# WGLab/NanoMod

Hardware: AMD Instinct MI355X
Metric: genomic positions/sec (KS + Stouffer) (higher is better)
Workload: dtype f32 keys / f64 p-values; 1 GPU; BASELINE.json configs[1]: E. coli 4.6 Mb: 4600000 positions in total (4600000 per GPU), 200 v 200 reads/position, KS + weighted Stouffer window=5; preset=ecoli, positions_total=4600000, positions_per_gpu=4600000, n0=200, n1=200, layout=fixed stride, ties=few, spread_milli=0, outlier_permille=0, rccl_ranks=0, ks_d=float form, bit for bit, parallelism=one GPU, no collective

## Files before the change

nanomod_amd/csrc/ks_rank.hpp:

```cpp
#pragma once
#include <hip/hip_runtime.h>
#include <stdint.h>
#include <type_traits>
#include "rank_stats_packed.hpp"
#include "packed_sort_i16.hpp"
#include "item_claim.hpp"

namespace nmod {

static __device__ const float kKsBig4[4] = {3.4028234663852886e38f, 3.4028234663852886e38f, 3.4028234663852886e38f, 3.4028234663852886e38f};
static __device__ const unsigned kKsInf4[4] = {0x7f800000u, 0x7f800000u, 0x7f800000u, 0x7f800000u};
static __device__ const unsigned kKsPad16[4] = {0x7fff7fffu, 0x7fff7fffu, 0x7fff7fffu, 0x7fff7fffu};

__host__ __device__ constexpr bool ks_packed_sort(int R, int LG, int DTYPE) { return DTYPE == 1 && R == 16 && (LG == 8 || LG == 16); }

template <int R, int LG>
struct KsLayout {
  static constexpr int C = R * LG;
  static constexpr int ROW = LG + 1;
  static constexpr int REGION = R * ROW;
  static constexpr int LAST = (R - 1) * ROW + LG - 1;
  static constexpr int END = LG;
  __device__ static __forceinline__ int word(int i) { return __mul24(i & (R - 1), ROW) + i / R; }
};

__host__ __device__ constexpr int ks_rank_pos_words(int R, int LG) {
  int w = 2 * R * (LG + 1);
  if (LG <= 16) while ((w & 31) != LG) ++w;
  return w;
}

template <typename T>
__device__ __forceinline__ T ks_global_load(const void* p) {
  typedef const T __attribute__((address_space(1)))* GlobalPtr;
  return *(GlobalPtr)(p);
}

typedef float KsF4v __attribute__((ext_vector_type(4)));
typedef short KsS4v __attribute__((ext_vector_type(4)));
typedef KsF4v KsF4 __attribute__((aligned(4)));
typedef KsS4v KsS4 __attribute__((aligned(2)));

template <int R, int LG, int DTYPE>
struct KsRows {
  using T = typename std::conditional<DTYPE == 0, float, int16_t>::type;
  using V4 = typename std::conditional<DTYPE == 0, KsF4, KsS4>::type;
  static constexpr int NK = R / 4;
  V4 v[NK];
  T s[3];

  __device__ __forceinline__ void request(const void* sig, int64_t off, int n, int gl) {
    const T* row = reinterpret_cast<const T*>(sig) + off;
    const T* dummy = ks_packed_sort(R, LG, DTYPE) ? reinterpret_cast<const T*>(kKsPad16) : reinterpret_cast<const T*>(kKsInf4);
    const bool long_row = n >= 4;
#pragma unroll
    for (int k = 0; k < NK; ++k) {
      const int idx = k * (4 * LG) + 4 * gl;
      const int t = n - idx;
      const T* p = (long_row && t > 0) ? row + ((t >= 4) ? idx : n - 4) : dummy;
      v[k] = ks_global_load<V4>(p);
    }
    s[0] = s[1] = s[2] = T(0);
    if (__ballot(!long_row && n > 0) != 0ull) {
#pragma unroll
      for (int e = 0; e < 3; ++e)
        if (!long_row && gl == 0 && e < n) s[e] = ks_global_load<T>(row + e);
    }
  }

  __device__ __forceinline__ void finish(float (&x)[R], int n, int gl) const {
    const float inf = __builtin_inff();
    const bool long_row = n >= 4;
#pragma unroll
    for (int k = 0; k < NK; ++k) {
      const int idx = k * (4 * LG) + 4 * gl;
      const int t = long_row ? n - idx : 0;
      if constexpr (DTYPE == 0) {
        x[4 * k + 0] = v[k].x; x[4 * k + 1] = v[k].y; x[4 * k + 2] = v[k].z; x[4 * k + 3] = v[k].w;
        if (__ballot(t > 0 && t < 4) != 0ull) {
          x[4 * k + 0] = (t >= 4 || t <= 0) ? x[4 * k + 0] : inf;
          x[4 * k + 1] = (t >= 3 || t <= 0) ? x[4 * k + 1] : inf;
          x[4 * k + 2] = (t >= 2 || t <= 0) ? x[4 * k + 2] : inf;
        }
      } else {
        x[4 * k + 0] = (t >= 4) ? (float)v[k].x : inf;
        x[4 * k + 1] = (t >= 3) ? (float)v[k].y : inf;
        x[4 * k + 2] = (t >= 2) ? (float)v[k].z : inf;
        x[4 * k + 3] = (t >= 1) ? (float)v[k].w : inf;
      }
    }
    if (__ballot(!long_row && n > 0) != 0ull) {
#pragma unroll
      for (int e = 0; e < 3; ++e) x[e] = (!long_row && gl == 0 && e < n) ? (float)s[e] : x[e];
    }
  }

  __device__ __forceinline__ void finish_packed(unsigned (&p)[8], int n, int gl) const {
    static_assert(R == 16, "packed rows: 16 keys per lane");
    const bool long_row = n >= 4;
#pragma unroll
    for (int k = 0; k < NK; ++k) {
      p[2 * k] = ((unsigned)(unsigned short)v[k].y << 16) | (unsigned)(unsigned short)v[k].x;
      p[2 * k + 1] = ((unsigned)(unsigned short)v[k].w << 16) | (unsigned)(unsigned short)v[k].z;
      const int idx = k * (4 * LG) + 4 * gl;
      const int t = long_row ? n - idx : 0;
      if (__ballot(t > 0 && t < 4) != 0ull) {
        if (t == 3) p[2 * k] = (p[2 * k] & 0xffff0000u) | 0x7fffu;
        if (t == 2 || t == 1) p[2 * k] = 0x7fff7fffu;
        if (t == 1) p[2 * k + 1] = (p[2 * k + 1] & 0xffff0000u) | 0x7fffu;
      }
    }
    if (__ballot(!long_row && n > 0) != 0ull) {
      if (!long_row && gl == 0) {
        const unsigned s0 = (0 < n) ? (unsigned)(unsigned short)s[0] : 0x7fffu;
        const unsigned s1 = (1 < n) ? (unsigned)(unsigned short)s[1] : 0x7fffu;
        const unsigned s2 = (2 < n) ? (unsigned)(unsigned short)s[2] : 0x7fffu;
        p[0] = (s1 << 16) | s0;
        p[1] = (0x7fffu << 16) | s2;
      }
    }
  }
};

template <int LG>
__device__ __forceinline__ unsigned seg_allmax_u32(unsigned v) {
  v = max(v, (unsigned)dpp_i<NMOD_QP(1, 0, 3, 2), 0xf, 0xf, true>(0, (int)v));
  v = max(v, (unsigned)dpp_i<NMOD_QP(2, 3, 0, 1), 0xf, 0xf, true>(0, (int)v));
  v = max(v, (unsigned)dpp_i<kDppRowHalfMirror, 0xf, 0xf, true>(0, (int)v));
  if constexpr (LG >= 16) v = max(v, (unsigned)dpp_i<kDppRowMirror, 0xf, 0xf, true>(0, (int)v));
  if constexpr (LG >= 32) v = max(v, (unsigned)__builtin_amdgcn_ds_swizzle((int)v, 0x401F));
  if constexpr (LG == 64) v = max(__builtin_amdgcn_readlane(v, 0), __builtin_amdgcn_readlane(v, 32));
  return v;
}

template <int LG>
__device__ __forceinline__ unsigned seg_exscan_add_u32(unsigned v, int gl) {
  unsigned inc = v;
  auto step = [&](auto tag, int dist) {
    constexpr int C = decltype(tag)::value;
    unsigned t = (unsigned)dpp_i<C, 0xf, 0xf, true>(0, (int)inc);
    inc += (gl >= dist) ? t : 0u;
  };
  step(std::integral_constant<int, kDppRowShr + 1>{}, 1);
  step(std::integral_constant<int, kDppRowShr + 2>{}, 2);
  step(std::integral_constant<int, kDppRowShr + 4>{}, 4);
  if constexpr (LG >= 16) step(std::integral_constant<int, kDppRowShr + 8>{}, 8);
  if constexpr (LG >= 32) {
    unsigned t = (unsigned)dpp_i<kDppRowBcast15, 0xA>(0, (int)inc);
    inc += ((gl & 16) != 0) ? t : 0u;
  }
  if constexpr (LG == 64) {
    unsigned t = (unsigned)dpp_i<kDppRowBcast31, 0xC>(0, (int)inc);
    inc += (gl >= 32) ? t : 0u;
  }
  return inc - v;
}

template <int R, int LG>
__device__ __forceinline__ void seg_sort_any(float (&x)[R], const LaneSel& sel, int lane) {
  seg_sort<R, (LG == 64 ? 32 : LG)>(x, sel, lane);
  if constexpr (LG == 64) merge_lanes<R, 64>(x, sel, lane);
}

template <int R, int LG, bool LE, bool FULL = true>
__device__ __forceinline__ const float* ks_search(const float* base, float x) {
  using Lay = KsLayout<R, LG>;
  const float* p = base;
  bool all = false;
  if constexpr (FULL) {
    const float last = base[Lay::LAST];
    all = LE ? (last <= x) : (last < x);
  }
#pragma unroll
  for (int hc = LG / 2; hc >= 1; hc >>= 1) {
    const float t = p[(R - 1) * Lay::ROW + hc - 1];
    const bool right = LE ? (t <= x) : (t < x);
    p = right ? p + hc : p;
  }
#pragma unroll
  for (int h = R / 2; h >= 1; h >>= 1) {
    const float t = p[(h - 1) * Lay::ROW];
    const bool right = LE ? (t <= x) : (t < x);
    p = right ? p + h * Lay::ROW : p;
  }
  return all ? base + Lay::END : p;
}

struct KsTops { float hi, lo0, lo1, last; };
template <int R, int LG>
__device__ __forceinline__ KsTops ks_tops(const float* base) {
  using Lay = KsLayout<R, LG>;
  auto uni = [](float v) { return __int_as_float(__builtin_amdgcn_readfirstlane(__float_as_int(v))); };
  KsTops t;
  t.hi = uni(base[(R - 1) * Lay::ROW + LG / 2 - 1]);
  t.lo0 = uni(base[(R - 1) * Lay::ROW + LG / 4 - 1]);
  t.lo1 = uni(base[(R - 1) * Lay::ROW + LG / 2 + LG / 4 - 1]);
  t.last = uni(base[Lay::LAST]);
  return t;
}
template <int R, int LG>
__device__ __forceinline__ const float* ks_search_tops(const float* base, float x, const KsTops& t) {
  using Lay = KsLayout<R, LG>;
  static_assert(LG >= 4, "two row levels");
  const bool all = t.last < x;
  const bool r1 = t.hi < x;
  const float t2 = r1 ? t.lo1 : t.lo0;
  const bool r2 = t2 < x;
  const float* p = base + (r1 ? LG / 2 : 0) + (r2 ? LG / 4 : 0);
#pragma unroll
  for (int hc = LG / 8; hc >= 1; hc >>= 1) {
    const float v = p[(R - 1) * Lay::ROW + hc - 1];
    p = (v < x) ? p + hc : p;
  }
#pragma unroll
  for (int h = R / 2; h >= 1; h >>= 1) {
    const float v = p[(h - 1) * Lay::ROW];
    p = (v < x) ? p + h * Lay::ROW : p;
  }
  return all ? base + Lay::END : p;
}

__device__ __forceinline__ double fmax_numbers(double a, double b) {
  double r;
  asm("v_max_f64 %0, %1, %2" : "=v"(r) : "v"(a), "v"(b));
  return r;
}

template <int LG>
__device__ __forceinline__ double seg_allmax_f64(double v) {
  v = fmax_numbers(v, dpp_f64_row(v, 0)); v = fmax_numbers(v, dpp_f64_row(v, 1)); v = fmax_numbers(v, dpp_f64_row(v, 2));
  if constexpr (LG >= 16) v = fmax_numbers(v, dpp_f64_row(v, 3));
  if constexpr (LG >= 32) v = fmax(v, xor16_f64(v));
  if constexpr (LG == 64) v = wave_max_f64(v);
  return v;
}

__device__ __forceinline__ double hist_exact_quot(int c, double n, double r) {
  const double dc = (double)c;
  const double q0 = __dmul_rn(dc, r);
  const double rem = __fma_rn(-q0, n, dc);
  return __fma_rn(rem, r, q0);
}

template <int LG>
__device__ __forceinline__ void seg_moments_packed16(const unsigned (&p)[8], int n, int gl, double& mean, double& m2, double rcp_n = 0.0) {
  int s1 = 0;
  double s2 = 0.0;
#pragma unroll
  for (int j = 0; j < 8; ++j) {
    const int lo = (int)(short)(p[j] & 0xffffu), hi = (int)p[j] >> 16;
    s1 += lo + hi;
    const double dl = (double)lo, dh = (double)hi;
    s2 = __fma_rn(dl, dl, s2);
    s2 = __fma_rn(dh, dh, s2);
  }
  int valid = 0;
#pragma unroll
  for (int k = 0; k < 4; ++k) valid += min(max(n - (k * 4 * LG + 4 * gl), 0), 4);
  valid = (n >= 4) ? valid : ((gl == 0) ? n : 0);
  const int npad = 16 - valid;
  s1 -= 32767 * npad;
  s2 -= 1073676289.0 * (double)npad;
  unsigned v = (unsigned)s1;
  v += (unsigned)dpp_i<NMOD_QP(1, 0, 3, 2), 0xf, 0xf, true>(0, (int)v);
  v += (unsigned)dpp_i<NMOD_QP(2, 3, 0, 1), 0xf, 0xf, true>(0, (int)v);
  v += (unsigned)dpp_i<kDppRowHalfMirror, 0xf, 0xf, true>(0, (int)v);
  if constexpr (LG >= 16) v += (unsigned)dpp_i<kDppRowMirror, 0xf, 0xf, true>(0, (int)v);
  const double S1 = (double)(int)v;
  const double S2 = seg_allsum_f64<LG>(s2);
  const double dn = (double)n;
  const double num = __fma_rn(dn, S2, -S1 * S1);
  const double rn = (rcp_n != 0.0) ? rcp_n : 1.0 / dn;
  mean = S1 * rn * 1e-3;
  m2 = num * rn * 1e-6;
}

template <int R, int LG, int DTYPE, bool FLAGS = false>
__global__ __launch_bounds__(64 * kWavesPerBlock, (R <= 16 ? 4 : 2))
void ks_rank_kernel(RankStatsArgs args) {
  static_assert(LG == 8 || LG == 16 || LG == 32 || LG == 64, "lanes per sorted group");
  static_assert(R >= 8 && R <= 32 && (R & (R - 1)) == 0, "registers per lane");
  constexpr int PW = 64 / LG;
  using Lay = KsLayout<R, LG>;
  constexpr int ROW = Lay::ROW;
  constexpr int POS_WORDS = ks_rank_pos_words(R, LG);
  constexpr int HIST_OFF = Lay::REGION;
  extern __shared__ __attribute__((aligned(16))) float lds_all[];

  const int lane = threadIdx.x & 63;
  const int wave = __builtin_amdgcn_readfirstlane(threadIdx.x >> 6);
  const int gl = lane & (LG - 1);
  const int slot = lane / LG;
  float* keys = lds_all + (wave * PW + slot) * POS_WORDS;
  unsigned* hist = reinterpret_cast<unsigned*>(keys + HIST_OFF);
  const int e0 = gl * R;

  const float inf = __builtin_inff();
  LaneSel sel;
#pragma unroll
  for (int b = 0; b < 6; ++b) sel.s[b] = ((lane >> b) & 1) ? inf : -inf;
  for (int r = gl; r < R; r += LG) keys[r * ROW + Lay::END] = inf;
  const bool uniform = args.stride0 > 0 && args.stride1 > 0;
  double* recip = reinterpret_cast<double*>(lds_all + kWavesPerBlock * PW * POS_WORDS);
  if (uniform && threadIdx.x == 0) {
    const int64_t a0 = args.stride0 < args.stride1 ? args.stride0 : args.stride1;
    const int64_t a1 = args.stride0 < args.stride1 ? args.stride1 : args.stride0;
    recip[0] = 1.0 / (double)a0; recip[1] = 1.0 / (double)a1;
  }
  __syncthreads();

  int64_t count = args.npos;
  const int32_t* list = nullptr;
  if (args.alt_gates != nullptr && args.alt_gates[args.class_id] != 0) {
    count = args.alt_meta[args.class_id];
    list = args.alt_list + args.alt_meta[kClassStride + args.class_id];
  } else if (args.pos_list) {
    count = args.class_meta[args.class_id];
    list = args.pos_list + args.class_meta[kClassStride + args.class_id];
  }
  const int64_t items = (count + PW - 1) / PW;
  const int64_t wave_global = (int64_t)blockIdx.x * kWavesPerBlock + wave;
  const int64_t wave_stride = (int64_t)gridDim.x * kWavesPerBlock;

  struct Item { bool valid, swap; int m, q; int64_t pos, off_s, off_q; };
  const uint32_t items32 = (uint32_t)items;
  auto describe = [&](uint32_t it) {
    Item d;
    const uint32_t li = min(it, items32) * PW + slot;
    d.valid = li < (uint32_t)count;
    d.pos = d.valid ? (list ? (int64_t)list[li] : (int64_t)li) : 0;
    int64_t o0 = 0, o1 = 0; int n0 = 0, n1 = 0;
    if (d.valid) {
      if (args.stride0 > 0) { o0 = (int64_t)((uint64_t)(uint32_t)d.pos * (uint64_t)(uint32_t)args.stride0); n0 = (int)args.stride0; }
      else { o0 = args.off0[d.pos]; n0 = (int)(args.off0[d.pos + 1] - o0); }
      if (args.stride1 > 0) { o1 = (int64_t)((uint64_t)(uint32_t)d.pos * (uint64_t)(uint32_t)args.stride1); n1 = (int)args.stride1; }
      else { o1 = args.off1[d.pos]; n1 = (int)(args.off1[d.pos + 1] - o1); }
    }
    d.swap = n1 < n0;
    d.m = d.swap ? n1 : n0; d.q = d.swap ? n0 : n1;
    d.off_s = d.swap ? o1 : o0; d.off_q = d.swap ? o0 : o1;
    return d;
  };
  const float big = 3.4028234663852886e38f;
  using Q4Raw = typename std::conditional<DTYPE == 0, KsF4, KsS4>::type;
  using Q1Raw = typename std::conditional<DTYPE == 0, float, int16_t>::type;
  auto load_q4 = [&](const void* sig, int64_t off, int idx, bool have) -> Q4Raw {
    using T = Q1Raw;
    const T* src = have ? reinterpret_cast<const T*>(sig) + off + idx : reinterpret_cast<const T*>(kKsBig4);
    return ks_global_load<Q4Raw>(src);
  };
  auto q4_values = [&](float (&xq)[4], const Q4Raw& t, bool have) {
    if constexpr (DTYPE == 0) {
      (void)have;
      xq[0] = t.x; xq[1] = t.y; xq[2] = t.z; xq[3] = t.w;
    } else {
      xq[0] = have ? (float)t.x : big; xq[1] = have ? (float)t.y : big;
      xq[2] = have ? (float)t.z : big; xq[3] = have ? (float)t.w : big;
    }
  };
  auto load_q1 = [&](const void* sig, int64_t off, int idx, bool have) -> Q1Raw {
    using T = Q1Raw;
    return ks_global_load<T>(have ? reinterpret_cast<const T*>(sig) + off + idx : reinterpret_cast<const T*>(kKsBig4));
  };
  auto q1_value = [&](Q1Raw v, bool have) -> float {
    if constexpr (DTYPE == 0) { (void)have; return v; }
    else return have ? (float)v : big;
  };

  ItemWalk walk;
  const uint32_t it_first = walk.begin(item_claim_plan<uint32_t>((uint32_t)items, (uint32_t)wave_stride, args.strided_items != 0),
                                      (uint32_t)wave_global, (uint32_t)wave_stride, args.claim + args.class_id, lane);
  Item cur = describe(it_first);
  constexpr bool PACKED = ks_packed_sort(R, LG, DTYPE);
  float x[R];
  unsigned pk[8];
  {
    KsRows<R, LG, DTYPE> first;
    first.request(cur.swap ? args.sig1 : args.sig0, cur.off_s, cur.m, gl);
    if constexpr (PACKED) first.finish_packed(pk, cur.m, gl);
    else first.finish(x, cur.m, gl);
  }
  __builtin_amdgcn_s_waitcnt(0x0F70);
  walk.collect();

  for (uint32_t it = it_first, it_next; it < items32; it = it_next) {
    const bool valid = cur.valid;
    const int64_t pos = cur.pos;
    const int m = cur.m, q = cur.q;
    const void* sig_q = cur.swap ? args.sig0 : args.sig1;
    const int64_t off_q = cur.off_q;

    const int full = q / (4 * LG);
    const int tail = (q - full * (4 * LG) + LG - 1) / LG;
    int full_w = full, tail_w = tail;
    if constexpr (PW > 1) {
      full_w = 0; tail_w = 0;
#pragma unroll
      for (int s = 0; s < PW; ++s) {
        full_w = max(full_w, __builtin_amdgcn_readlane(full, s * LG));
        tail_w = max(tail_w, __builtin_amdgcn_readlane(tail, s * LG));
      }
    } else {
      full_w = __builtin_amdgcn_readfirstlane(full);
      tail_w = __builtin_amdgcn_readfirstlane(tail);
    }
    int slots = (full_w * 4 + tail_w) * LG;
    bool coop = false;
    if constexpr (PW > 1) {
      int coop_cost = 0;
#pragma unroll
      for (int sl = 0; sl < PW; ++sl) {
        const int qs = __builtin_amdgcn_readlane(q, sl * LG);
        const int fs = qs / 256;
        coop_cost += fs * 4 + (qs - fs * 256 + 63) / 64;
      }
      coop = coop_cost < full_w * 4 + tail_w;
    }
    it_next = walk.next(it, lane);
    const Item nxt = describe(it_next);
    KsRows<R, LG, DTYPE> rows_next;
    rows_next.request(nxt.swap ? args.sig1 : args.sig0, nxt.off_s, nxt.m, gl);
    constexpr bool PIPE_COOP = LG == 8;
    auto row_of_slot = [&](int sl, const void*& sg, int64_t& of, int& qn) {
      const int src = sl * LG;
      auto rl64 = [&](unsigned long long v) {
        const unsigned lo = (unsigned)__builtin_amdgcn_readlane((int)(unsigned)v, src);
        const unsigned hi = (unsigned)__builtin_amdgcn_readlane((int)(unsigned)(v >> 32), src);
        return ((unsigned long long)hi << 32) | (unsigned long long)lo;
      };
      sg = reinterpret_cast<const void*>((uintptr_t)rl64((unsigned long long)(uintptr_t)sig_q));
      of = (int64_t)rl64((unsigned long long)off_q);
      qn = __builtin_amdgcn_readlane(q, src);
    };
    const void* sig_c = sig_q; int64_t off_c = off_q; int q_c = q;
    int idx_a = 4 * gl, idx_t = full * (4 * LG) + gl;
    bool have_a = !coop && 0 < full, have_t = !coop && idx_t < q;
    if constexpr (PIPE_COOP) {
      if (coop) {
        row_of_slot(0, sig_c, off_c, q_c);
        idx_a = 4 * lane; idx_t = (q_c / 256) * 256 + lane; have_a = q_c >= 256; have_t = idx_t < q_c;
      }
    }
    Q4Raw ra = load_q4(sig_c, off_c, idx_a, have_a);
    Q1Raw rt = load_q1(sig_c, off_c, idx_t, have_t);

    if constexpr (PACKED) {
      seg_sort_packed16<LG>(pk, lane);
      unpack_sorted16<LG>(pk, x);
    } else {
      seg_sort_any<R, LG>(x, sel, lane);
    }
#pragma unroll
    for (int r = 0; r < R; ++r) keys[r * ROW + gl] = x[r];
    if constexpr (PACKED) {
      const int real = m - e0;
#pragma unroll
      for (int r = 0; r < R; ++r)
        if (r >= real) keys[r * ROW + gl] = inf;
    }
#pragma unroll
    for (int r = 0; r < R; ++r) hist[r * ROW + gl] = 0u;
    if (gl == LG - 1) hist[Lay::END] = 0u;
    __builtin_amdgcn_fence(__ATOMIC_RELEASE, "wavefront");
    __builtin_amdgcn_wave_barrier();

    const bool s_full = __ballot(m == Lay::C) != 0ull;

    auto rank_and_count = [&](auto nv_tag, auto full_tag, const float* kbase, const float* xq) {
      constexpr int NV = decltype(nv_tag)::value;
      constexpr bool FULL = decltype(full_tag)::value;
      const float* lp[NV];
#pragma unroll
      for (int e = 0; e < NV; ++e) lp[e] = ks_search<R, LG, false, FULL>(kbase, xq[e]);
      unsigned inc[NV];
#pragma unroll
      for (int e = 0; e < NV; ++e) inc[e] = (*lp[e] == xq[e]) ? 0x10001u : 0x10000u;
#pragma unroll
      for (int e = 0; e < NV; ++e) atomicAdd(reinterpret_cast<unsigned*>(const_cast<float*>(lp[e])) + HIST_OFF, inc[e]);
    };

    [[maybe_unused]] auto rank_and_count_tops = [&](auto nv_tag, const float* kbase, const KsTops& tops, const float* xq) {
      constexpr int NV = decltype(nv_tag)::value;
      const float* lp[NV];
#pragma unroll
      for (int e = 0; e < NV; ++e) lp[e] = ks_search_tops<R, LG>(kbase, xq[e], tops);
      unsigned inc[NV];
#pragma unroll
      for (int e = 0; e < NV; ++e) inc[e] = (*lp[e] == xq[e]) ? 0x10001u : 0x10000u;
#pragma unroll
      for (int e = 0; e < NV; ++e) atomicAdd(reinterpret_cast<unsigned*>(const_cast<float*>(lp[e])) + HIST_OFF, inc[e]);
    };

    __builtin_amdgcn_s_waitcnt(0x0F70);
    walk.collect();
    if (!coop) {
#pragma unroll 1
      for (int c = 0; c < full_w; ++c) {
        const Q4Raw rb = load_q4(sig_q, off_q, (c + 1) * (4 * LG) + 4 * gl, c + 1 < full);
        float xa[4];
        q4_values(xa, ra, c < full);
        if (s_full) rank_and_count(std::integral_constant<int, 4>{}, std::true_type{}, keys, xa);
        else rank_and_count(std::integral_constant<int, 4>{}, std::false_type{}, keys, xa);
        ra = rb;
      }
#pragma unroll 1
      for (int c = 0; c < tail_w; ++c) {
        float xq[1] = {q1_value(rt, full * (4 * LG) + c * LG + gl < q)};
        const int idx = full * (4 * LG) + (c + 1) * LG + gl;
        rt = load_q1(sig_q, off_q, idx, idx < q);
        if (s_full) rank_and_count(std::integral_constant<int, 1>{}, std::true_type{}, keys, xq);
        else rank_and_count(std::integral_constant<int, 1>{}, std::false_type{}, keys, xq);
      }
    } else {
      const int cfull = q / 256;
      slots = (cfull * 4 + (q - cfull * 256 + 63) / 64) * 64;
      if constexpr (PIPE_COOP) {
#pragma unroll 1
      for (int sl = 0; sl < PW; ++sl) {
        const void* sig_n = sig_c; int64_t off_n = off_c; int q_n = 0;
        if (sl + 1 < PW) row_of_slot(sl + 1, sig_n, off_n, q_n);
        const int nfs = q_n / 256;
        const Q4Raw na = load_q4(sig_n, off_n, 4 * lane, nfs > 0);
        const Q1Raw nt = load_q1(sig_n, off_n, nfs * 256 + lane, nfs * 256 + lane < q_n);
        const float* kb = lds_all + (wave * PW + sl) * POS_WORDS;
        const int fs = q_c / 256, ts = (q_c - fs * 256 + 63) / 64;
        const KsTops tops = ks_tops<R, LG>(kb);
#pragma unroll 2
        for (int c = 0; c < fs; ++c) {
          const Q4Raw rb = load_q4(sig_c, off_c, min(c + 1, fs - 1) * 256 + 4 * lane, true);
          float xq[4];
          q4_values(xq, ra, true);
          rank_and_count_tops(std::integral_constant<int, 4>{}, kb, tops, xq);
          ra = rb;
        }
#pragma unroll 1
        for (int c = 0; c < ts; ++c) {
          const int idx_now = fs * 256 + c * 64 + lane;
          const Q1Raw r1 = load_q1(sig_c, off_c, idx_now + 64, idx_now + 64 < q_c);
          float xq[1] = {q1_value(rt, idx_now < q_c)};
          rank_and_count_tops(std::integral_constant<int, 1>{}, kb, tops, xq);
          rt = r1;
        }
        sig_c = sig_n; off_c = off_n; q_c = q_n; ra = na; rt = nt;
      }
      } else {
#pragma unroll 1
      for (int sl = 0; sl < PW; ++sl) {
        const int src = sl * LG;
        const int qs = __builtin_amdgcn_readlane(q, src);
        const unsigned long long sp = (unsigned long long)(uintptr_t)sig_q;
        auto rl64 = [&](unsigned long long v) {
          const unsigned lo = (unsigned)__builtin_amdgcn_readlane((int)(unsigned)v, src);
          const unsigned hi = (unsigned)__builtin_amdgcn_readlane((int)(unsigned)(v >> 32), src);
          return ((unsigned long long)hi << 32) | (unsigned long long)lo;
        };
        const void* sigs = reinterpret_cast<const void*>((uintptr_t)rl64(sp));
        const int64_t offs = (int64_t)rl64((unsigned long long)off_q);
        const float* kb = lds_all + (wave * PW + sl) * POS_WORDS;
        const int fs = qs / 256, ts = (qs - fs * 256 + 63) / 64;
#pragma unroll 1
        for (int c = 0; c < fs; ++c) {
          const int idx = c * 256 + 4 * lane;
          float xq[4];
          q4_values(xq, load_q4(sigs, offs, idx, true), true);
          rank_and_count(std::integral_constant<int, 4>{}, std::true_type{}, kb, xq);
        }
#pragma unroll 1
        for (int c = 0; c < ts; ++c) {
          const int idx = fs * 256 + c * 64 + lane;
          float xq[1] = {q1_value(load_q1(sigs, offs, idx, idx < qs), idx < qs)};
          rank_and_count(std::integral_constant<int, 1>{}, std::true_type{}, kb, xq);
        }
      }
      }
    }
    __builtin_amdgcn_fence(__ATOMIC_RELEASE, "wavefront");
    __builtin_amdgcn_wave_barrier();
    if (gl == 0) { const unsigned extra = (unsigned)(slots - q); hist[Lay::word(m)] -= extra << 16; }
    __builtin_amdgcn_fence(__ATOMIC_RELEASE, "wavefront");
    __builtin_amdgcn_wave_barrier();

    unsigned h[R];
#pragma unroll
    for (int r = 0; r < R - 1; ++r) h[r] = hist[(r + 1) * ROW + gl];
    h[R - 1] = hist[gl + 1];
    const unsigned h0 = hist[0];
    unsigned tot = 0;
#pragma unroll
    for (int r = 0; r < R; ++r) tot += h[r];
    const unsigned cum = seg_exscan_add_u32<LG>(tot, gl) + h0;
    unsigned best = 0;
    float s_own[R];
#pragma unroll
    for (int r = 0; r < R; ++r) s_own[r] = keys[r * ROW + gl];
    const float s_next = keys[gl + 1];
    const bool tie_lane = ((tot | h0) & 0xffffu) != 0u;
    bool slow = __ballot(tie_lane) != 0ull;
    if (!slow) {
      float gap = inf;
#pragma unroll
      for (int r = 0; r < R; ++r) gap = fminf(gap, ((r == R - 1) ? s_next : s_own[r + 1]) - s_own[r]);
      slow = __ballot(gap == 0.0f) != 0ull;
    }
    if (!slow) {
      const int kq_max = __mul24(m - 1, q);
      int kq = min(__mul24(e0, q), kq_max);
      const int cmax = q - (int)(hist[Lay::word(m)] >> 16);
      int c = min((int)(cum >> 16), cmax);
      int a = __mul24(c, m) - kq;
      int hi = (gl == 0) ? a : -(1 << 30), lo = 1 << 30;
      if (gl == 0) hist[0] = (unsigned)c;
#pragma unroll
      for (int r = 0; r < R; ++r) {
        lo = min(lo, a);
        c = min(c + (int)(h[r] >> 16), cmax);
        if (r < R - 1) hist[(r + 1) * ROW + gl] = (unsigned)c; else hist[gl + 1] = (unsigned)c;
        kq = min(kq + q, kq_max);
        a = __mul24(c, m) - kq;
        hi = max(hi, a);
      }
      best = (unsigned)max(max(hi, q - lo), 0);
    } else {
      int cl = (int)(cum >> 16);
      int hi = (gl == 0) ? __mul24((int)(h0 >> 16) - (int)(h0 & 0xffffu), m) : 0, lo = 0;
      const int nkq_min = -__mul24(m, q);
      int nkq = -__mul24(e0, q);
#pragma unroll
      for (int r = 0; r < R; ++r) {
        const float up = (r == R - 1) ? s_next : s_own[r + 1];
        const bool run_end = s_own[r] != up;
        nkq = max(nkq - q, nkq_min);
        const int cand_b = __mul24(cl, m) + nkq;
        lo = min(lo, cand_b);
        const int clp = cl;
        cl += (int)(h[r] >> 16);
        const int cu = cl - (int)(h[r] & 0xffffu);
        {
          unsigned short* w16 = reinterpret_cast<unsigned short*>(hist + ((r < R - 1) ? (r + 1) * ROW + gl : gl + 1));
          w16[0] = (unsigned short)cu; w16[1] = (unsigned short)clp;
        }
        const int cand_a = __mul24(cu, m) + nkq;
        hi = max(hi, run_end ? cand_a : 0);
      }
      best = (unsigned)max(hi, -lo);
    }
    const unsigned lbest = best;
    best = seg_allmax_u32<LG>(best);
    double dmax = 0.0;
    if (!args.ks_rational_d) {
      constexpr int BPL = (R + LG - 1) / LG;
      const double dm = (double)m, dq = (double)q;
      double rm, rq;
      if (uniform) { rm = recip[0]; rq = recip[1]; }
      else { rm = 1.0 / dm; rq = 1.0 / dq; }
      const int seg_base = lane & ~(LG - 1);
      const unsigned long long hits = __ballot(lbest == best && best != 0u);
      using Mine = typename std::conditional<LG == 64, unsigned long long, unsigned>::type;
      Mine mine = (Mine)(hits >> seg_base);
      if constexpr (LG < 32) mine &= (Mine)((1u << LG) - 1u);
      if (gl == 0 && (mine & (Mine)1)) {
        const int cu0 = (int)(h0 >> 16) - (int)(h0 & 0xffffu);
        if ((unsigned)__mul24(cu0, m) == best) dmax = hist_exact_quot(cu0, dq, rq);
      }
      __builtin_amdgcn_fence(__ATOMIC_RELEASE, "wavefront");
      __builtin_amdgcn_wave_barrier();
      unsigned pw = 0u;
      unsigned long long parked = 0ull;
      auto flush = [&]() {
        const double d = fabs(hist_exact_quot((int)(pw >> 16), dm, rm) - hist_exact_quot((int)(pw & 0xffffu), dq, rq));
        dmax = (d > dmax) ? d : dmax;
        pw = 0u; parked = 0ull;
      };
      const int ibest = (int)best;
      const int nq = -q;
      const int t_shift = slow ? 16 : 0;
      const unsigned t_mask = slow ? 0xffffu : 0xffffffffu;
#pragma unroll 1
      for (;;) {
        const unsigned long long m_act = __ballot(mine != (Mine)0);
        if (m_act == 0ull) break;
        const bool act = mine != (Mine)0;
        int hl = act ? (__ffsll((long long)mine) - 1) : 0;
        asm volatile("" : "+v"(hl));
        mine &= mine - (Mine)1;
#pragma unroll 1
        for (int j = 0; j < BPL; ++j) {
          const int rr = gl * BPL + j;
          const bool in = rr < R;
          const int k = hl * R + rr + 1;
          const int wp = in ? rr * ROW + hl : 0;
          const int wk = in ? ((rr + 1 < R) ? (rr + 1) * ROW + hl : hl + 1) : 0;
          const unsigned tp = hist[wp], tk = hist[wk];
          const float key_p = keys[wp], key_k = keys[wk];
          const int clp = (int)((slow ? tk : tp) >> t_shift);
          const int cu = (int)(tk & t_mask);
          const int nkq = __mul24(k, nq);
          const int cand_b = __mul24(clp, m) + nkq;
          const int cand_a = __mul24(cu, m) + nkq;
          const bool ok = act && in && key_p != key_k;
          const bool hb = ok && (cand_b == ibest || cand_b == -ibest);
          const bool ha = ok && (cand_a == ibest || cand_a == -ibest) && !(hb && cu == clp);
          const unsigned kw = (unsigned)k << 16;
          if constexpr (LG < 64) {
            unsigned long long m_ok = m_act & __ballot(key_p != key_k);
            if constexpr (BPL * LG != R) m_ok &= __ballot(rr < R);
            const unsigned long long m_b = m_ok & (__ballot(cand_b == ibest) | __ballot(cand_b == -ibest));
            const unsigned long long m_a = m_ok & (__ballot(cand_a == ibest) | __ballot(cand_a == -ibest)) & (~m_b | __ballot(cu != clp));
            if ((m_b & parked) != 0ull) flush();
            pw = hb ? (kw | (unsigned)clp) : pw; parked |= m_b;
            if ((m_a & parked) != 0ull) flush();
            pw = ha ? (kw | (unsigned)cu) : pw; parked |= m_a;
          } else {
            if (__ballot(hb && pw != 0u) != 0ull) flush();
            pw = hb ? (kw | (unsigned)clp) : pw;
            if (__ballot(ha && pw != 0u) != 0ull) flush();
            pw = ha ? (kw | (unsigned)cu) : pw;
          }
        }
      }
      if ((LG < 64) ? (parked != 0ull) : (__ballot(pw != 0u) != 0ull)) flush();
      dmax = seg_allmax_f64<LG>(dmax);
    }
    if (valid && gl == 0) {
      args.ks_num[pos] = (m > 0 && q > 0) ? best : 0u;
      args.ks_d_ref[pos] = (m > 0 && q > 0) ? dmax : 0.0;
    }
    if constexpr (FLAGS) {
      const unsigned t = seg_allmax_u32<LG>(tie_lane ? 1u : 0u);
      if (valid && gl == 0) args.tied[pos] = (uint8_t)t;
    }
    __builtin_amdgcn_wave_barrier();
    __builtin_amdgcn_s_waitcnt(0x0F70);
    if constexpr (PACKED) rows_next.finish_packed(pk, nxt.m, gl);
    else rows_next.finish(x, nxt.m, gl);
    cur = nxt;
  }
}

}
```

nanomod_amd/csrc/rank_stats_inst.hip:

```cpp
#include <algorithm>
#include <atomic>
#include "rank_stats.hpp"
#include "rank_stats_packed.hpp"
#include "ks_rank.hpp"
#include "rank_all.hpp"
#include "rank_hist.hpp"
#include "rank_count.hpp"
#include "rank_count_wide.hpp"
#include "rank_count_value.hpp"
#include "rank_stats_launch.hpp"

#ifndef NMOD_INST_DTYPE
#error "define NMOD_INST_DTYPE and NMOD_INST_ALL"
#endif

namespace nmod {

namespace {
constexpr int DT = NMOD_INST_DTYPE;
constexpr bool ALL = NMOD_INST_ALL != 0;
using KernelFn = void (*)(RankStatsArgs);

#if NMOD_INST_ALL
template <int C0, int C1>
constexpr KernelFn kernel_of() { return rank_pair_kernel<(1 << C0), (1 << C1), DT>; }

template <int C0>
KernelFn pick1(int c1) {
  switch (c1) {
    case 0: return kernel_of<C0, 0>();
    case 1: return kernel_of<C0, 1>();
    case 2: return kernel_of<C0, 2>();
    case 3: return kernel_of<C0, 3>();
    case 4: return kernel_of<C0, 4>();
    default: return kernel_of<C0, 5>();
  }
}
KernelFn pick(int c0, int c1) {
  switch (c0) {
    case 0: return pick1<0>(c1);
    case 1: return pick1<1>(c1);
    case 2: return pick1<2>(c1);
    case 3: return pick1<3>(c1);
    case 4: return pick1<4>(c1);
    default: return pick1<5>(c1);
  }
}
KernelFn pick_wide(int cmin) {
  switch (cmin) {
    case 0: return rank_hist_kernel<1, 64, DT, true>;
    case 1: return rank_hist_kernel<2, 64, DT, true>;
    default: return rank_hist_kernel<4, 64, DT, true>;
  }
}
KernelFn pick_packed(int cm, bool after_count) {
  if (after_count) return rank_hist_kernel<16, 16, DT, false, true>;
  switch (cm) {
    case 0: return rank_hist_kernel<8, 8, DT>;
    case 1: return rank_hist_kernel<16, 8, DT>;
    case 2: return rank_hist_kernel<16, 16, DT>;
    case 3: return rank_hist_kernel<16, 32, DT>;
    default: return rank_hist_kernel<16, 64, DT>;
  }
}
#else
KernelFn pick_ks(int cs, bool flags) {
#if NMOD_INST_DTYPE == 0
  if (flags) {
    switch (cs) {
      case 0: return ks_rank_kernel<8, 8, DT, true>;
      case 1: return ks_rank_kernel<16, 8, DT, true>;
      case 2: return ks_rank_kernel<16, 16, DT, true>;
      case 3: return ks_rank_kernel<16, 32, DT, true>;
      case 4: return ks_rank_kernel<16, 64, DT, true>;
      default: return ks_rank_kernel<32, 64, DT, true>;
    }
  }
#endif
  (void)flags;
  switch (cs) {
    case 0: return ks_rank_kernel<8, 8, DT>;
    case 1: return ks_rank_kernel<16, 8, DT>;
    case 2: return ks_rank_kernel<16, 16, DT>;
    case 3: return ks_rank_kernel<16, 32, DT>;
    case 4: return ks_rank_kernel<16, 64, DT>;
    default: return ks_rank_kernel<32, 64, DT>;
  }
}
#endif

hipError_t blocks_per_cu(std::atomic<int>* slot, const void* fn, size_t lds, int* per_cu, size_t lds_limit = 0) {
  int pc = slot ? slot->load(std::memory_order_relaxed) : 0;
  if (pc <= 0) {
    hipError_t e = hipFuncSetAttribute(fn, hipFuncAttributeMaxDynamicSharedMemorySize, (int)(lds_limit ? lds_limit : lds));
    if (e != hipSuccess) return e;
    e = hipOccupancyMaxActiveBlocksPerMultiprocessor(&pc, fn, 64 * kWavesPerBlock, lds);
    if (e != hipSuccess) return e;
    if (pc < 1) return hipErrorLaunchOutOfResources;
    if (slot) slot->store(pc, std::memory_order_relaxed);
  }
  *per_cu = pc;
  return hipSuccess;
}
constexpr int kCacheDevices = 64;
int cache_device() {
  int dev = 0;
  return hipGetDevice(&dev) == hipSuccess && dev >= 0 && dev < kCacheDevices ? dev : -1;
}
int64_t grid_of(int64_t work_items, int num_cus, int per_cu) {
  return std::max<int64_t>(1, std::min<int64_t>((work_items + kWavesPerBlock - 1) / kWavesPerBlock, (int64_t)num_cus * per_cu));
}

hipError_t launch_rank_stats(int cls, int num_cus, int64_t work_items, hipStream_t stream, const RankStatsArgs& args) {
  const bool ks = cls >= kKsClassBase && cls < kNumClasses;
  const bool packed = cls >= kNumGeneralClasses && cls < kKsClassBase;
  KernelFn fn = nullptr;
#if NMOD_INST_ALL
  if (ks) return hipErrorInvalidValue;
  const bool wide = wide_class(cls);
  const bool counting = packed && cls - kNumGeneralClasses == 2 && args.cnt_gate != nullptr && args.cnt_done != nullptr;
  fn = packed ? pick_packed(cls - kNumGeneralClasses, counting)
       : wide ? pick_wide(wide_class_of_s(cls))
              : pick(cls / kNumSizeClasses, cls % kNumSizeClasses);
#else
  if (!ks) return hipErrorInvalidValue;
  fn = pick_ks(cls - kKsClassBase, args.tied != nullptr);
#endif
  const size_t lds = rank_stats_lds_bytes(cls, ALL, DT);
  if (ks || packed) {
    const int pw = ks ? ksonly_positions_per_wave(cls - kKsClassBase) : packed_positions_per_wave(cls - kNumGeneralClasses);
    work_items = (work_items + pw - 1) / pw;
  }
  static std::atomic<int> per_cu_cache[kCacheDevices][2 * kClassStride];
  const int dev = cache_device();
#if NMOD_INST_ALL
  const int slot_id = cls + (counting ? kClassStride : 0);
  const size_t lds_limit = wide ? rank_stats_lds_bytes(kWideBigBase + wide_class_of_s(cls), ALL, DT) : lds;
#else
  const int slot_id = cls + ((ks && args.tied) ? kClassStride : 0);
  const size_t lds_limit = lds;
#endif
  int per_cu = 0;
  hipError_t e = blocks_per_cu(dev >= 0 ? &per_cu_cache[dev][slot_id] : nullptr, reinterpret_cast<const void*>(fn), lds, &per_cu, lds_limit);
  if (e != hipSuccess) return e;
#if NMOD_INST_ALL
  if (counting) {
    CntProbeArgs pa;
    pa.sig0 = args.sig0; pa.sig1 = args.sig1; pa.off0 = args.off0; pa.off1 = args.off1; pa.stride0 = args.stride0; pa.stride1 = args.stride1;
    pa.npos = args.npos; pa.pos_list = args.pos_list; pa.class_meta = args.class_meta; pa.class_id = args.class_id; pa.dtype = DT; pa.gate = args.cnt_gate;
#if NMOD_INST_DTYPE == 0
    const bool int_keys = args.tied != nullptr;
    if (int_keys) hipLaunchKernelGGL(cnt_probe_kernel<2>, dim3(1), dim3(1024), 0, stream, pa);
    else hipLaunchKernelGGL(cnt_probe_kernel<0>, dim3(1), dim3(1024), 0, stream, pa);
    static std::atomic<int> cnt_per_cu[kCacheDevices][2];
    KernelFn cfn = int_keys ? (KernelFn)rank_count_kernel<2> : (KernelFn)rank_count_kernel<0>;
    std::atomic<int>* cslot = dev >= 0 ? &cnt_per_cu[dev][int_keys ? 1 : 0] : nullptr;
#else
    hipLaunchKernelGGL(cnt_probe_kernel<DT>, dim3(1), dim3(1024), 0, stream, pa);
    static std::atomic<int> cnt_per_cu[kCacheDevices][1];
    KernelFn cfn = rank_count_kernel<DT>;
    std::atomic<int>* cslot = dev >= 0 ? &cnt_per_cu[dev][0] : nullptr;
#endif
    const size_t clds = rank_count_lds_bytes();
    int cpc = 0;
    e = blocks_per_cu(cslot, reinterpret_cast<const void*>(cfn), clds, &cpc);
    if (e != hipSuccess) return e;
    hipLaunchKernelGGL(cfn, dim3((unsigned)grid_of(work_items, num_cus, cpc)), dim3(64 * kWavesPerBlock), clds, stream, args);
    e = hipGetLastError();
    if (e != hipSuccess) return e;
  }
#endif
  const int64_t blocks = grid_of(work_items, num_cus, per_cu);
#if NMOD_INST_ALL
  if (counting) {
    RankStatsArgs a2 = args;
    a2.cnt_mode = 1;
    KernelFn plain = pick_packed(cls - kNumGeneralClasses, false);
    static std::atomic<int> plain_per_cu[kCacheDevices];
    int ppc = 0;
    e = blocks_per_cu(dev >= 0 ? &plain_per_cu[dev] : nullptr, reinterpret_cast<const void*>(plain), lds, &ppc);
    if (e != hipSuccess) return e;
    hipLaunchKernelGGL(plain, dim3((unsigned)blocks), dim3(64 * kWavesPerBlock), lds, stream, a2);
    a2.cnt_mode = 2;
    hipLaunchKernelGGL(fn, dim3((unsigned)blocks), dim3(64 * kWavesPerBlock), lds, stream, a2);
    return hipGetLastError();
  }
#endif
  hipLaunchKernelGGL(fn, dim3((unsigned)blocks), dim3(64 * kWavesPerBlock), lds, stream, args);
  return hipGetLastError();
}

hipError_t count_wide_prepare(const int* classes, int nclasses, hipStream_t stream, const RankStatsArgs& a, const CountWideWs& w) {
  if (nclasses <= 0) return hipSuccess;
  if (nclasses > kClassStride) return hipErrorInvalidValue;
  CntWideProbeArgs pa;
  pa.sig0 = a.sig0; pa.sig1 = a.sig1; pa.off0 = a.off0; pa.off1 = a.off1; pa.stride0 = a.stride0; pa.stride1 = a.stride1; pa.npos = a.npos;
  pa.pos_list = a.pos_list; pa.class_meta = a.class_meta; pa.nclasses = nclasses; pa.gate = w.gates; pa.segs = w.gates + kClassStride; pa.work_meta = w.work_meta; pa.min_q = NMOD_INST_ALL ? 0 : kCwKsMinQ;
  for (int i = 0; i < nclasses && i < kClassStride; ++i) { pa.cls[i] = classes[i]; pa.max_s[i] = 64 << count_wide_rs_index(classes[i]); }
  hipError_t e = hipMemsetAsync(w.gates, 0, kClassStride * 4, stream);
  if (e != hipSuccess) return e;
#if NMOD_INST_DTYPE == 0
  if (a.tied != nullptr) hipLaunchKernelGGL(HIP_KERNEL_NAME(cnt_wide_probe_kernel<2, NMOD_INST_ALL == 0>), dim3((unsigned)nclasses), dim3(1024), 0, stream, pa);
  else hipLaunchKernelGGL(HIP_KERNEL_NAME(cnt_wide_probe_kernel<0, NMOD_INST_ALL == 0>), dim3((unsigned)nclasses), dim3(1024), 0, stream, pa);
#else
  hipLaunchKernelGGL(HIP_KERNEL_NAME(cnt_wide_probe_kernel<1, NMOD_INST_ALL == 0>), dim3((unsigned)nclasses), dim3(1024), 0, stream, pa);
#endif
  return hipGetLastError();
}

hipError_t count_wide_run(int num_cus, int64_t work_items, hipStream_t stream, const RankStatsArgs& a, const CountWideWs& w, bool value_class) {
  typedef void (*CwFn)(CntWideArgs);
#if NMOD_INST_DTYPE == 0
  const bool int_keys = a.tied != nullptr;
  CwFn fn = int_keys ? (CwFn)rank_count_wide_kernel<2, NMOD_INST_ALL == 0> : (CwFn)rank_count_wide_kernel<0, NMOD_INST_ALL == 0>;
  CwFn vfn = int_keys ? (CwFn)rank_count_value_kernel<2, NMOD_INST_ALL == 0> : (CwFn)rank_count_value_kernel<0, NMOD_INST_ALL == 0>;
  const int slot = int_keys ? 1 : 0;
#else
  CwFn fn = (CwFn)rank_count_wide_kernel<1, NMOD_INST_ALL == 0>;
  CwFn vfn = (CwFn)rank_count_value_kernel<1, NMOD_INST_ALL == 0>;
  const int slot = 0;
#endif
  static std::atomic<int> per_cu[kCacheDevices][2], vper_cu[kCacheDevices][2];
  const int dev = cache_device();
  const size_t lds = rank_count_wide_lds_bytes();
  int pc = 0;
  hipError_t e = blocks_per_cu(dev >= 0 ? &per_cu[dev][slot] : nullptr, reinterpret_cast<const void*>(fn), lds, &pc);
  if (e != hipSuccess) return e;
  CntWideArgs ca;
  ca.rs = a; ca.gates = w.gates; ca.segs = w.gates + kClassStride; ca.work_list = w.work_list; ca.work_meta = w.work_meta;
  hipLaunchKernelGGL(fn, dim3((unsigned)grid_of(work_items, num_cus, pc)), dim3(64 * kWavesPerBlock), lds, stream, ca);
  if (value_class) {
    const size_t vlds = rank_count_value_lds_bytes();
    int vpc = 0;
    e = blocks_per_cu(dev >= 0 ? &vper_cu[dev][slot] : nullptr, reinterpret_cast<const void*>(vfn), vlds, &vpc);
    if (e != hipSuccess) return e;
    hipLaunchKernelGGL(vfn, dim3((unsigned)grid_of(work_items, num_cus, vpc)), dim3(64 * kWavesPerBlock), vlds, stream, ca);
  }
  return hipGetLastError();
}
}

#define NMOD_CAT2(a, b) a##b
#define NMOD_CAT(a, b) NMOD_CAT2(a, b)
#define NMOD_K1_NAME NMOD_CAT(NMOD_CAT(k1_d, NMOD_INST_DTYPE), NMOD_CAT(_a, NMOD_INST_ALL))
const K1Launcher& NMOD_K1_NAME() {
  static const K1Launcher k1 = {launch_rank_stats, count_wide_prepare, count_wide_run};
  return k1;
}

}
```

Before: 1.454 billion positions/s.

## Add uniform-stride KS kernel specialization with scalarized row sizes

Adds a UNIFORM template instance of the KS rank kernel, chosen when both strides are fixed and there is no position list, alt gates or tie tracking. In that instance the per-item descriptor drops the offset and list lookups, row load offsets are precomputed once, and the row sizes are kept in scalar registers so the ballot-based tail checks, cooperative-slot accounting and per-iteration reciprocal loads disappear. The aim is to cut per-position VALU and branch overhead on the fixed-stride layout, at the cost of another set of kernel instantiations and heavy reliance on inline-asm register hints.

```diff
diff --git a/nanomod_amd/csrc/ks_rank.hpp b/nanomod_amd/csrc/ks_rank.hpp
--- a/nanomod_amd/csrc/ks_rank.hpp
+++ b/nanomod_amd/csrc/ks_rank.hpp
@@ -68,16 +68,51 @@
     }
   }
 
+  struct Plan { unsigned boff[NK]; int last; bool last_live; };
+  __device__ static __forceinline__ Plan plan(int n, int gl) {
+    Plan pl;
+    pl.last = (n >= 4) ? (n - 1) / (4 * LG) : -1;
+    pl.last_live = n >= 4 && n - (pl.last * (4 * LG) + 4 * gl) > 0;
+#pragma unroll
+    for (int k = 0; k < NK; ++k) {
+      const int idx = k * (4 * LG) + 4 * gl;
+      const int t = n - idx;
+      pl.boff[k] = (n >= 4 && t > 0) ? (unsigned)((t >= 4) ? idx : n - 4) * (unsigned)sizeof(T) : 0u;
+    }
+    return pl;
+  }
+  __device__ __forceinline__ void request_uniform(const void* sig, int64_t off, int n, int gl, const Plan& pl) {
+    const char* row = reinterpret_cast<const char*>(reinterpret_cast<const T*>(sig) + off);
+    const char* dummy = ks_packed_sort(R, LG, DTYPE) ? reinterpret_cast<const char*>(kKsPad16) : reinterpret_cast<const char*>(kKsInf4);
+    int last = pl.last;
+    asm volatile("" : "+s"(last));
+#pragma unroll
+    for (int k = 0; k < NK; ++k) {
+      const bool live = k < last || (k == last && pl.last_live);
+      v[k] = ks_global_load<V4>(live ? row + pl.boff[k] : dummy);
+    }
+    s[0] = s[1] = s[2] = T(0);
+    asm volatile("" : "+v"(gl), "+s"(n));
+    if (n < 4) {
+#pragma unroll
+      for (int e = 0; e < 3; ++e)
+        if (gl == 0 && e < n) s[e] = ks_global_load<T>(reinterpret_cast<const T*>(row) + e);
+    }
+  }
+
+  template <bool UNI = false>
   __device__ __forceinline__ void finish(float (&x)[R], int n, int gl) const {
     const float inf = __builtin_inff();
+    if constexpr (UNI) asm volatile("" : "+v"(gl), "+s"(n));
     const bool long_row = n >= 4;
+    const bool row_end = long_row && (n & 3) != 0;
 #pragma unroll
     for (int k = 0; k < NK; ++k) {
       const int idx = k * (4 * LG) + 4 * gl;
       const int t = long_row ? n - idx : 0;
       if constexpr (DTYPE == 0) {
         x[4 * k + 0] = v[k].x; x[4 * k + 1] = v[k].y; x[4 * k + 2] = v[k].z; x[4 * k + 3] = v[k].w;
-        if (__ballot(t > 0 && t < 4) != 0ull) {
+        if (UNI ? row_end : (__ballot(t > 0 && t < 4) != 0ull)) {
           x[4 * k + 0] = (t >= 4 || t <= 0) ? x[4 * k + 0] : inf;
           x[4 * k + 1] = (t >= 3 || t <= 0) ? x[4 * k + 1] : inf;
           x[4 * k + 2] = (t >= 2 || t <= 0) ? x[4 * k + 2] : inf;
@@ -89,28 +124,31 @@
         x[4 * k + 3] = (t >= 1) ? (float)v[k].w : inf;
       }
     }
-    if (__ballot(!long_row && n > 0) != 0ull) {
+    if (UNI ? !long_row : (__ballot(!long_row && n > 0) != 0ull)) {
 #pragma unroll
       for (int e = 0; e < 3; ++e) x[e] = (!long_row && gl == 0 && e < n) ? (float)s[e] : x[e];
     }
   }
 
+  template <bool UNI = false>
   __device__ __forceinline__ void finish_packed(unsigned (&p)[8], int n, int gl) const {
     static_assert(R == 16, "packed rows: 16 keys per lane");
+    if constexpr (UNI) asm volatile("" : "+v"(gl), "+s"(n));
     const bool long_row = n >= 4;
+    const bool row_end = long_row && (n & 3) != 0;
 #pragma unroll
     for (int k = 0; k < NK; ++k) {
       p[2 * k] = ((unsigned)(unsigned short)v[k].y << 16) | (unsigned)(unsigned short)v[k].x;
       p[2 * k + 1] = ((unsigned)(unsigned short)v[k].w << 16) | (unsigned)(unsigned short)v[k].z;
       const int idx = k * (4 * LG) + 4 * gl;
       const int t = long_row ? n - idx : 0;
-      if (__ballot(t > 0 && t < 4) != 0ull) {
+      if (UNI ? row_end : (__ballot(t > 0 && t < 4) != 0ull)) {
         if (t == 3) p[2 * k] = (p[2 * k] & 0xffff0000u) | 0x7fffu;
         if (t == 2 || t == 1) p[2 * k] = 0x7fff7fffu;
         if (t == 1) p[2 * k + 1] = (p[2 * k + 1] & 0xffff0000u) | 0x7fffu;
       }
     }
-    if (__ballot(!long_row && n > 0) != 0ull) {
+    if (UNI ? !long_row : (__ballot(!long_row && n > 0) != 0ull)) {
       if (!long_row && gl == 0) {
         const unsigned s0 = (0 < n) ? (unsigned)(unsigned short)s[0] : 0x7fffu;
         const unsigned s1 = (1 < n) ? (unsigned)(unsigned short)s[1] : 0x7fffu;
@@ -275,9 +313,10 @@
   m2 = num * rn * 1e-6;
 }
 
-template <int R, int LG, int DTYPE, bool FLAGS = false>
+template <int R, int LG, int DTYPE, bool FLAGS = false, bool UNIFORM = false>
 __global__ __launch_bounds__(64 * kWavesPerBlock, (R <= 16 ? 4 : 2))
 void ks_rank_kernel(RankStatsArgs args) {
+  static_assert(!(UNIFORM && FLAGS), "the float64 front end keeps the generic instance");
   static_assert(LG == 8 || LG == 16 || LG == 32 || LG == 64, "lanes per sorted group");
   static_assert(R >= 8 && R <= 32 && (R & (R - 1)) == 0, "registers per lane");
   constexpr int PW = 64 / LG;
@@ -311,6 +350,9 @@
 
   int64_t count = args.npos;
   const int32_t* list = nullptr;
+  if constexpr (UNIFORM) {
+    if (count <= 0) return;
+  } else
   if (args.alt_gates != nullptr && args.alt_gates[args.class_id] != 0) {
     count = args.alt_meta[args.class_id];
     list = args.alt_list + args.alt_meta[kClassStride + args.class_id];
@@ -324,10 +366,21 @@
 
   struct Item { bool valid, swap; int m, q; int64_t pos, off_s, off_q; };
   const uint32_t items32 = (uint32_t)items;
+  const bool u_swap = args.stride1 < args.stride0;
+  const int u_m = (int)(u_swap ? args.stride1 : args.stride0), u_q = (int)(u_swap ? args.stride0 : args.stride1);
+  const void* const u_sig_s = u_swap ? args.sig1 : args.sig0;
+  const void* const u_sig_q = u_swap ? args.sig0 : args.sig1;
   auto describe = [&](uint32_t it) {
     Item d;
     const uint32_t li = min(it, items32) * PW + slot;
     d.valid = li < (uint32_t)count;
+    if constexpr (UNIFORM) {
+      d.pos = d.valid ? (int64_t)li : 0;
+      d.swap = u_swap; d.m = u_m; d.q = u_q;
+      d.off_s = (int64_t)((uint64_t)(uint32_t)d.pos * (uint64_t)(uint32_t)u_m);
+      d.off_q = (int64_t)((uint64_t)(uint32_t)d.pos * (uint64_t)(uint32_t)u_q);
+      return d;
+    }
     d.pos = d.valid ? (list ? (int64_t)list[li] : (int64_t)li) : 0;
     int64_t o0 = 0, o1 = 0; int n0 = 0, n1 = 0;
     if (d.valid) {
@@ -374,11 +427,25 @@
   constexpr bool PACKED = ks_packed_sort(R, LG, DTYPE);
   float x[R];
   unsigned pk[8];
+  [[maybe_unused]] typename KsRows<R, LG, DTYPE>::Plan row_plan;
+  if constexpr (UNIFORM) row_plan = KsRows<R, LG, DTYPE>::plan(u_m, gl);
+  [[maybe_unused]] double u_dm = 0.0, u_dq = 0.0, u_rm = 0.0, u_rq = 0.0;
+  if constexpr (UNIFORM) {
+    auto uni64 = [](double v) {
+      const unsigned long long b = (unsigned long long)__double_as_longlong(v);
+      unsigned lo, hi;
+      asm("v_readfirstlane_b32 %0, %1" : "=s"(lo) : "v"((unsigned)b));
+      asm("v_readfirstlane_b32 %0, %1" : "=s"(hi) : "v"((unsigned)(b >> 32)));
+      return __longlong_as_double((long long)(((unsigned long long)hi << 32) | lo));
+    };
+    u_dm = uni64((double)u_m); u_dq = uni64((double)u_q); u_rm = uni64(recip[0]); u_rq = uni64(recip[1]);
+  }
   {
     KsRows<R, LG, DTYPE> first;
-    first.request(cur.swap ? args.sig1 : args.sig0, cur.off_s, cur.m, gl);
-    if constexpr (PACKED) first.finish_packed(pk, cur.m, gl);
-    else first.finish(x, cur.m, gl);
+    if constexpr (UNIFORM) first.request_uniform(u_sig_s, cur.off_s, u_m, gl, row_plan);
+    else first.request(cur.swap ? args.sig1 : args.sig0, cur.off_s, cur.m, gl);
+    if constexpr (PACKED) first.template finish_packed<UNIFORM>(pk, cur.m, gl);
+    else first.template finish<UNIFORM>(x, cur.m, gl);
   }
   __builtin_amdgcn_s_waitcnt(0x0F70);
   walk.collect();
@@ -386,14 +453,15 @@
   for (uint32_t it = it_first, it_next; it < items32; it = it_next) {
     const bool valid = cur.valid;
     const int64_t pos = cur.pos;
-    const int m = cur.m, q = cur.q;
-    const void* sig_q = cur.swap ? args.sig0 : args.sig1;
+    const int m = UNIFORM ? u_m : cur.m, q = UNIFORM ? u_q : cur.q;
+    const void* sig_q = UNIFORM ? u_sig_q : (cur.swap ? args.sig0 : args.sig1);
     const int64_t off_q = cur.off_q;
 
     const int full = q / (4 * LG);
     const int tail = (q - full * (4 * LG) + LG - 1) / LG;
     int full_w = full, tail_w = tail;
-    if constexpr (PW > 1) {
+    if constexpr (UNIFORM) {
+    } else if constexpr (PW > 1) {
       full_w = 0; tail_w = 0;
 #pragma unroll
       for (int s = 0; s < PW; ++s) {
@@ -406,7 +474,8 @@
     }
     int slots = (full_w * 4 + tail_w) * LG;
     bool coop = false;
-    if constexpr (PW > 1) {
+    if constexpr (UNIFORM) {
+    } else if constexpr (PW > 1) {
       int coop_cost = 0;
 #pragma unroll
       for (int sl = 0; sl < PW; ++sl) {
@@ -419,7 +488,8 @@
     it_next = walk.next(it, lane);
     const Item nxt = describe(it_next);
     KsRows<R, LG, DTYPE> rows_next;
-    rows_next.request(nxt.swap ? args.sig1 : args.sig0, nxt.off_s, nxt.m, gl);
+    if constexpr (UNIFORM) rows_next.request_uniform(u_sig_s, nxt.off_s, u_m, gl, row_plan);
+    else rows_next.request(nxt.swap ? args.sig1 : args.sig0, nxt.off_s, nxt.m, gl);
     constexpr bool PIPE_COOP = LG == 8;
     auto row_of_slot = [&](int sl, const void*& sg, int64_t& of, int& qn) {
       const int src = sl * LG;
@@ -453,7 +523,8 @@
 #pragma unroll
     for (int r = 0; r < R; ++r) keys[r * ROW + gl] = x[r];
     if constexpr (PACKED) {
-      const int real = m - e0;
+      int real = m - e0;
+      if constexpr (UNIFORM) asm volatile("" : "+v"(real));
 #pragma unroll
       for (int r = 0; r < R; ++r)
         if (r >= real) keys[r * ROW + gl] = inf;
@@ -464,7 +535,9 @@
     __builtin_amdgcn_fence(__ATOMIC_RELEASE, "wavefront");
     __builtin_amdgcn_wave_barrier();
 
-    const bool s_full = __ballot(m == Lay::C) != 0ull;
+    int m_full = m;
+    if constexpr (UNIFORM) asm volatile("" : "+s"(m_full));
+    const bool s_full = UNIFORM ? (m_full == Lay::C) : (__ballot(m == Lay::C) != 0ull);
 
     auto rank_and_count = [&](auto nv_tag, auto full_tag, const float* kbase, const float* xq) {
       constexpr int NV = decltype(nv_tag)::value;
@@ -496,7 +569,8 @@
     if (!coop) {
 #pragma unroll 1
       for (int c = 0; c < full_w; ++c) {
-        const Q4Raw rb = load_q4(sig_q, off_q, (c + 1) * (4 * LG) + 4 * gl, c + 1 < full);
+        const Q4Raw rb = UNIFORM ? load_q4(sig_q, off_q, min(c + 1, full - 1) * (4 * LG) + 4 * gl, true)
+                                 : load_q4(sig_q, off_q, (c + 1) * (4 * LG) + 4 * gl, c + 1 < full);
         float xa[4];
         q4_values(xa, ra, c < full);
         if (s_full) rank_and_count(std::integral_constant<int, 4>{}, std::true_type{}, keys, xa);
@@ -603,8 +677,11 @@
       slow = __ballot(gap == 0.0f) != 0ull;
     }
     if (!slow) {
-      const int kq_max = __mul24(m - 1, q);
+      int m_ev = m;
+      if constexpr (UNIFORM) asm volatile("" : "+s"(m_ev));
+      const int kq_max = __mul24(m_ev - 1, q);
       int kq = min(__mul24(e0, q), kq_max);
+      if constexpr (UNIFORM) asm volatile("" : "+v"(kq));
       const int cmax = q - (int)(hist[Lay::word(m)] >> 16);
       int c = min((int)(cum >> 16), cmax);
       int a = __mul24(c, m) - kq;
@@ -623,8 +700,11 @@
     } else {
       int cl = (int)(cum >> 16);
       int hi = (gl == 0) ? __mul24((int)(h0 >> 16) - (int)(h0 & 0xffffu), m) : 0, lo = 0;
-      const int nkq_min = -__mul24(m, q);
+      int m_ev = m;
+      if constexpr (UNIFORM) asm volatile("" : "+s"(m_ev));
+      const int nkq_min = -__mul24(m_ev, q);
       int nkq = -__mul24(e0, q);
+      if constexpr (UNIFORM) asm volatile("" : "+v"(nkq));
 #pragma unroll
       for (int r = 0; r < R; ++r) {
         const float up = (r == R - 1) ? s_next : s_own[r + 1];
@@ -649,9 +729,10 @@
     double dmax = 0.0;
     if (!args.ks_rational_d) {
       constexpr int BPL = (R + LG - 1) / LG;
-      const double dm = (double)m, dq = (double)q;
+      const double dm = UNIFORM ? u_dm : (double)m, dq = UNIFORM ? u_dq : (double)q;
       double rm, rq;
-      if (uniform) { rm = recip[0]; rq = recip[1]; }
+      if constexpr (UNIFORM) { rm = u_rm; rq = u_rq; }
+      else if (uniform) { rm = recip[0]; rq = recip[1]; }
       else { rm = 1.0 / dm; rq = 1.0 / dq; }
       const int seg_base = lane & ~(LG - 1);
       const unsigned long long hits = __ballot(lbest == best && best != 0u);
@@ -722,8 +803,8 @@
       dmax = seg_allmax_f64<LG>(dmax);
     }
     if (valid && gl == 0) {
-      args.ks_num[pos] = (m > 0 && q > 0) ? best : 0u;
-      args.ks_d_ref[pos] = (m > 0 && q > 0) ? dmax : 0.0;
+      args.ks_num[pos] = (UNIFORM || (m > 0 && q > 0)) ? best : 0u;
+      args.ks_d_ref[pos] = (UNIFORM || (m > 0 && q > 0)) ? dmax : 0.0;
     }
     if constexpr (FLAGS) {
       const unsigned t = seg_allmax_u32<LG>(tie_lane ? 1u : 0u);
@@ -731,8 +812,8 @@
     }
     __builtin_amdgcn_wave_barrier();
     __builtin_amdgcn_s_waitcnt(0x0F70);
-    if constexpr (PACKED) rows_next.finish_packed(pk, nxt.m, gl);
-    else rows_next.finish(x, nxt.m, gl);
+    if constexpr (PACKED) rows_next.template finish_packed<UNIFORM>(pk, nxt.m, gl);
+    else rows_next.template finish<UNIFORM>(x, nxt.m, gl);
     cur = nxt;
   }
 }
diff --git a/nanomod_amd/csrc/rank_stats_inst.hip b/nanomod_amd/csrc/rank_stats_inst.hip
--- a/nanomod_amd/csrc/rank_stats_inst.hip
+++ b/nanomod_amd/csrc/rank_stats_inst.hip
@@ -64,7 +64,7 @@
   }
 }
 #else
-KernelFn pick_ks(int cs, bool flags) {
+KernelFn pick_ks(int cs, bool flags, bool uniform) {
 #if NMOD_INST_DTYPE == 0
   if (flags) {
     switch (cs) {
@@ -78,6 +78,16 @@
   }
 #endif
   (void)flags;
+  if (uniform) {
+    switch (cs) {
+      case 0: return ks_rank_kernel<8, 8, DT, false, true>;
+      case 1: return ks_rank_kernel<16, 8, DT, false, true>;
+      case 2: return ks_rank_kernel<16, 16, DT, false, true>;
+      case 3: return ks_rank_kernel<16, 32, DT, false, true>;
+      case 4: return ks_rank_kernel<16, 64, DT, false, true>;
+      default: return ks_rank_kernel<32, 64, DT, false, true>;
+    }
+  }
   switch (cs) {
     case 0: return ks_rank_kernel<8, 8, DT>;
     case 1: return ks_rank_kernel<16, 8, DT>;
@@ -124,20 +134,21 @@
               : pick(cls / kNumSizeClasses, cls % kNumSizeClasses);
 #else
   if (!ks) return hipErrorInvalidValue;
-  fn = pick_ks(cls - kKsClassBase, args.tied != nullptr);
+  const bool ks_uniform = args.tied == nullptr && args.stride0 > 0 && args.stride1 > 0 && args.pos_list == nullptr && args.alt_gates == nullptr;
+  fn = pick_ks(cls - kKsClassBase, args.tied != nullptr, ks_uniform);
 #endif
   const size_t lds = rank_stats_lds_bytes(cls, ALL, DT);
   if (ks || packed) {
     const int pw = ks ? ksonly_positions_per_wave(cls - kKsClassBase) : packed_positions_per_wave(cls - kNumGeneralClasses);
     work_items = (work_items + pw - 1) / pw;
   }
-  static std::atomic<int> per_cu_cache[kCacheDevices][2 * kClassStride];
+  static std::atomic<int> per_cu_cache[kCacheDevices][3 * kClassStride];
   const int dev = cache_device();
 #if NMOD_INST_ALL
   const int slot_id = cls + (counting ? kClassStride : 0);
   const size_t lds_limit = wide ? rank_stats_lds_bytes(kWideBigBase + wide_class_of_s(cls), ALL, DT) : lds;
 #else
-  const int slot_id = cls + ((ks && args.tied) ? kClassStride : 0);
+  const int slot_id = cls + ((ks && args.tied) ? kClassStride : ks_uniform ? 2 * kClassStride : 0);
   const size_t lds_limit = lds;
 #endif
   int per_cu = 0;
```

Result: faster. 1.491 billion positions/s, median of 6 (+2.5%).
